# andrewhou1/BlindShadowRemoval

Hardware: AMD Instinct MI355X
Metric: images/sec at 256x256 batch inference (GSC generator forward) (higher is better)
Workload: dtype f32; 1 GPU; BASELINE configs[1]: batch=32 synthetic 256x256x3 per GPU, full GSC generator fp32 (seeded random-init weights in the ckpt-94 variable layout); global_batch=32, height=256, width=256, parallelism=dp1, forwards_in_flight=1, collective=none

## Files before the change

### blindshadowremoval_amd/_lib.py

```python
from __future__ import annotations

import ctypes
import os
from typing import Optional

from . import build as _build
from .build import LIB_PATH

ABI_VERSION = 8
NUM_CLASSES = 7
CLASS_NAMES = ("conv3x3", "convT3x3", "conv1x1", "attention", "conv7", "glue", "convT3x3_ni2")

_lib: Optional[ctypes.CDLL] = None

c_i, c_v, c_sz, c_s = ctypes.c_int, ctypes.c_void_p, ctypes.c_size_t, ctypes.c_char_p
_BS = [c_i, c_i]
_BLOBS = [c_v, c_sz, c_v, c_sz]

SIGNATURES = {
    "bsr_abi_version": (c_i, None),
    "bsr_last_error": (c_s, None),
    "bsr_source_sha": (c_s, None),
    "bsr_create": (c_i, [ctypes.POINTER(c_v), c_i, c_v, c_sz, c_i]),
    "bsr_destroy": (None, [c_v]),
# ... 3 lines not shown
    "bsr_forward_rgb": (c_i, [c_v, c_v, c_v, c_i, c_i, c_i, c_v, c_v]),
    "bsr_workspace_bytes": (c_sz, [c_i, c_i, c_i]),
    "bsr_handle_workspace_bytes": (c_sz, [c_v, c_i, c_i, c_i]),
    "bsr_reserve": (c_i, [c_v, c_i, c_i, c_i]),
    "bsr_probe": (c_i, [c_v, c_s, c_v, c_sz, ctypes.POINTER(c_i * 4), c_v]),
    "bsr_set_timing": (c_i, [c_v, c_i]),
    "bsr_get_timing": (c_i, [c_v, ctypes.POINTER(ctypes.c_float * NUM_CLASSES), ctypes.POINTER(c_i * NUM_CLASSES)]),
    "bsr_timing_launches": (c_i, [c_v]),
    "bsr_timing_entry": (c_i, [c_v, c_i, c_s, c_sz, ctypes.POINTER(ctypes.c_float), ctypes.POINTER(c_i)]),
    "bsr_clock_trace": (c_i, [c_i, c_v, c_i, c_i, c_v, c_v, c_v]),
    "bsr_check_range": (c_i, [c_v, c_v]),
    "bsr_peek_range": (c_i, [c_v]),
    "bsr_debug_attention": (c_i, [c_v, c_v, c_i, c_i, c_v]),
    "bsr_debug_attention_rgb": (c_i, [c_v, c_v, c_i, c_i, c_v]),
    "bsr_debug_attention_dtype": (c_i, [c_v, c_v, c_i, c_i, c_i, c_v]),
    "bsr_debug_attention_qw": (c_i, [c_v, c_v, c_i, c_i, c_i, c_v]),
    "bsr_debug_attention_split": (c_i, [c_v, c_v, c_i, c_i, c_i, c_v]),
    "bsr_debug_attention_kv1": (c_i, [c_v, c_v, c_i, c_i, c_i, c_v]),
    "bsr_debug_split_qkv": (c_i, [c_v, c_v, c_i, c_i, c_v]),
    "bsr_debug_wino_conv": (c_i, [c_v, c_v, c_v, c_v, c_i, c_i, c_i, c_i, c_v]),
    "bsr_debug_wino_filter": (c_i, [c_v, c_v]),
    "bsr_debug_wino_convt": (c_i, [c_v, c_v, c_v, c_v, c_i, c_i, c_i, c_i, c_i, c_i, c_i, c_i, c_v]),
    "bsr_debug_wino_convt_filter": (c_i, [c_v, c_v, c_i]),
    "bsr_debug_keys_compose": (c_i, [c_v, c_v, c_v, c_v]),
    "bsr_debug_values_compose": (c_i, [c_v, c_v, c_v, c_v, c_v, c_v]),
    "bsr_prep_rows": (c_i, [c_i, c_v, c_sz, c_sz, c_sz, c_i, c_i, c_v, c_v, c_v]),
    "bsr_prep_groups": (c_i, [c_i, c_v, c_sz, c_sz, c_sz, c_i, c_i, c_i, c_v, c_v, c_v]),
    "bsr_png_unfilter": (c_i, [c_i, c_v, c_sz, c_sz, c_i, c_v]),
    "bsr_png_unfilter_tall": (c_i, [c_i, c_v, c_sz, c_sz, c_i, c_v]),
    "bsr_png_file_bytes": (c_sz, [c_i, c_i]),
    "bsr_png_scratch_bytes": (c_sz, [c_i]),
    "bsr_png_encode": (c_i, [c_i, c_v, c_i, c_i, c_i, c_v, c_sz, c_v, c_v]),
    "bsr_png_encode_figs": (c_i, [c_i, c_i, c_v, c_v, c_v, c_v, c_v, c_v, c_i, c_i, c_i, c_v, c_sz, c_v, c_v]),
    "bsr_crop_faces": (c_i, [c_i, c_v, c_sz, c_sz, c_i, c_i, c_v]),
    "bsr_paste_faces": (c_i, [c_i, c_v, c_sz, c_sz, c_i, c_i, c_v, c_i, c_v, c_i, c_v, c_i, c_i, c_v]),
    "bsr_ucb_post_scratch_bytes": (c_sz, _BS),
    "bsr_ucb_post": (c_i, [c_i, c_v, c_v, c_v, c_i, c_i, c_v, c_v, c_v, c_v, c_v, c_v]),
    "bsr_ucb_post_rgb_scratch_bytes": (c_sz, _BS),
    "bsr_ucb_post_rgb": (c_i, [c_i, c_v, c_v, c_v, c_i, c_i, c_v, c_v, c_v, c_v, c_v, c_v]),
    "bsr_ucb_post_tsm_scratch_bytes": (c_sz, _BS),
    "bsr_ucb_post_tsm": (c_i, [c_i, c_v, c_v, c_v, c_i, c_i, c_v, c_v, c_v, c_v, c_v, c_v, c_v]),
    "bsr_sfw_score_scratch_bytes": (c_sz, _BS),
    "bsr_sfw_score": (c_i, [c_i, c_v, c_i, c_i, c_v, c_v, c_v, c_v, c_v, c_v, c_v]),
    "bsr_shadow_synth_scratch_bytes": (c_sz, _BS),
    "bsr_shadow_synth": (c_i, [c_i, c_v, c_v, c_v, c_v, c_v, c_sz, c_i, c_i, c_v, c_v, c_v, c_v, c_v, c_v, c_v]),
    "bsr_train_losses_scratch_bytes": (c_sz, _BS),
# ... 160 lines not shown
```

### blindshadowremoval_amd/csrc/bsr_api.hip

```cpp
#include "../../include/bsr_hip.h"

#include <hip/hip_runtime.h>
#include <stdint.h>
#include <stdio.h>
#include <stdlib.h>
#include <string.h>

#include <initializer_list>
#include <string>
#include <type_traits>
#include <unordered_map>
#include <vector>

#include "attention.h"
#include "attention256.h"
#include "attention_h16.h"
#include "conv3_f16.h"
#include "conv_n16.h"
#include "gemm_nloop.h"
#include "glue_kernels.h"
#include "igemm_conv.h"
#include "igemm_h16.h"
#include "png_kernels.h"
#include "prep_kernels.h"
#include "prep_group_kernels.h"
#include "rgb_head.h"
#include "stem7.h"
#include "ucb_kernels.h"
#include "ucb_rgb_kernels.h"
#include "ucb_tsm_kernels.h"
#include "sfw_kernels.h"
#include "wino_conv2.h"
#include "wino_convt.h"
#include "wild_crop_kernels.h"
#include "wild_paste_kernels.h"
#include "shadow_synth_kernels.h"
#include "train_losses_kernels.h"
#include "disc_kernels.h"
#include "disc_grad_kernels.h"
#include "disc_wgrad_kernels.h"
#include "clr_tail_grad_kernels.h"
#include "clr_up_grad_kernels.h"
#include "grey_up_grad_kernels.h"
#include "nonlocal_grad_kernels.h"
#include "bottleneck_grad_kernels.h"
#include "colour_trunk_grad_kernels.h"
#include "lower_trunk_grad_kernels.h"
#include "heads_grad_kernels.h"
#include "vgg_kernels.h"
#include "vgg_grad_kernels.h"

namespace {

thread_local std::string g_last_error;

int fail(int code, const std::string& msg) {
// ... 133 lines not shown
  for (int i = 0; i < v.nblk; ++i) p.r[i] = take(cells * (i < 3 ? v.cs_r : v.cs_h), !v.rgb);
  p.xh = take(cells * v.cs_h, true);
  p.ybuf = take(px * v.cs_y);
  p.qh = take(px * v.cs_qh);
  p.f1 = take(px2 / 16 * 128);
  p.f2 = take(px2 / 4 * 96);
  p.cf = take(px2 * CS_CF);
  p.probe = take(px2 / 64 * 2);
  p.reg32 = take(v.tsm ? cells * 4 : 0);
  p.share = take(v.tsm ? cells * 2 * v.c_r : 0);
  p.yh = take(px1 * 3);
  p.con = take(px1 * 3);
  p.total = off;
  return p;
}

}

struct bsr_handle {
  int device = 0;
  float* d_blob = nullptr;
  float* d_wino = nullptr;
  float* d_winot = nullptr;
  float* d_keys = nullptr;
  float* d_values = nullptr;
  float* att_scratch = nullptr;
  size_t att_scratch_floats = 0;
  std::unordered_map<std::string, LayerW> layers;
  Variant var = kGSC;
  int dtype = BSR_DTYPE_F32;
  float head_bias[2] = {0.f, 0.f};
  const float* tail_w = nullptr;
  const float* clr_gs_w = nullptr;
  float* ws = nullptr;
  size_t ws_floats = 0;
  Plan plan{};
  const float* rgb_tail_w = nullptr;
  const float* rgb_head_b = nullptr;
  int B = 0, H = 0, W = 0;
  bool ran = false;
  bool att_in_lds = false;
  unsigned* range_flag = nullptr;
  bool fuse_heads = true;
  bool conv1_gemm = true;
  bool att_pv1 = false;
  bool conv3_f16 = true;
  bool fuse_attw = true;
  bool wino_conv2 = true;
  bool wino_pairs = true;
  bool wino_convt = true;
  bool keys_conv2 = true;
  bool values_conv2 = true;
  bool att_is_o = false;
  bool timing = false;
  std::vector<hipEvent_t> ev;
  std::vector<int> ev_class;
  std::vector<std::string> ev_name;
  size_t ev_used = 0;
};

namespace {

const char* const kRangeMsg =
    "an activation exceeded the fp16 range (|x| >= 65520) in a forward of this 16-bit-mode handle: its outputs are not trustworthy "
    "(inf / NaN where the fp32 path stays finite).  Re-run those inputs on a BSR_DTYPE_F32 handle; bsr_check_range() clears the condition";

constexpr size_t kWinoFloats = 8 * 16 * 128 * 16;
void wino_filter_transform(const float* direct, float* out) {
  static const double G[4][3] = {{1.0, 0.0, 0.0}, {0.5, 0.5, 0.5}, {0.5, -0.5, 0.5}, {0.0, 0.0, 1.0}};
  for (int k = 0; k < 128; ++k)
    for (int n = 0; n < 128; ++n) {
      double t[4][3];
      for (int x = 0; x < 4; ++x)
// ... 13 lines not shown

constexpr int kWinoTLayers = 3;
const char* const kWinoTNames[kWinoTLayers] = {"up2", "up3", "clr_up3"};
constexpr int kWinoTCin[kWinoTLayers] = {160, 128, 96};
constexpr size_t wino_convt_floats(int cin) { return (size_t)(cin / 16) * 25 * 64 * 16; }
constexpr size_t wino_convt_offset(int layer) { return layer == 0 ? 0 : wino_convt_offset(layer - 1) + wino_convt_floats(kWinoTCin[layer - 1]); }
void wino_convt_filter_transform(const float* direct, float* out, int cin) {
  static const double G[5][3] = {{0.0, 1.0, 0.0}, {0.0, 1.0, 0.0}, {0.0, 0.0, 1.0}, {1.0, 0.0, 1.0}, {1.0, 0.0, 0.0}};
  for (int k = 0; k < cin; ++k)
    for (int n = 0; n < 64; ++n) {
      double t[5][3];
      for (int x = 0; x < 5; ++x)
        for (int b = 0; b < 3; ++b) {
          double acc = 0.0;
          for (int a = 0; a < 3; ++a) acc += G[x][a] * (double)direct[((size_t)((k / 32) * 9 + a * 3 + b) * 64 + n) * 36 + k % 32];
          t[x][b] = acc;
        }
      const int kk = k % 16, g = kk / 8, hh = (kk % 8) / 4, j = kk % 4;
      for (int x = 0; x < 5; ++x)
        for (int y = 0; y < 5; ++y) {
          double acc = 0.0;
          for (int b = 0; b < 3; ++b) acc += t[x][b] * G[y][b];
          out[(((((size_t)(k / 16) * 25 + 5 * x + y) * 2 + n / 32) * 2 + g) * 64 + 32 * hh + n % 32) * 4 + j] = (float)acc;
        }
    }
}

constexpr int kKeysN = 288 + 256, kKeysNPad = kKeysN + 64, kC3qNPad = 768;
constexpr size_t kKeysFloats = (size_t)4 * kKeysNPad * 36 + kKeysNPad;
void keys_compose(const float* c3q_w, const float* c3q_b, float* out_w, float* out_b) {
  auto src = [&](int k, int n) -> const float& { return c3q_w[((size_t)(k / 32) * kC3qNPad + n) * 36 + k % 32]; };
  memset(out_w, 0, (size_t)4 * kKeysNPad * 36 * sizeof(float));
  memset(out_b, 0, kKeysNPad * sizeof(float));
  for (int ch = 0; ch < 4; ++ch) {
    memcpy(out_w + (size_t)ch * kKeysNPad * 36, c3q_w + (size_t)ch * kC3qNPad * 36, (size_t)288 * 36 * sizeof(float));
    memcpy(out_w + ((size_t)ch * kKeysNPad + 416) * 36, c3q_w + ((size_t)ch * kC3qNPad + 544) * 36, (size_t)128 * 36 * sizeof(float));
  }
  memcpy(out_b, c3q_b, 288 * sizeof(float));
  memcpy(out_b + 416, c3q_b + 544, 128 * sizeof(float));
  for (int m = 0; m < 128; ++m) {
    for (int k = 0; k < 128; ++k) {
      double acc = 0.0;
      for (int c = 0; c < 128; ++c) acc += (double)src(k, 288 + c) * (double)src(m, 416 + c);
      out_w[((size_t)(k / 32) * kKeysNPad + 288 + m) * 36 + k % 32] = (float)acc;
    }
    double acc = 0.0;
// ... 301 lines not shown
    end();
    if (fuse) return;
    begin(K_GLUE, "heads_post");
    hipLaunchKernelGGL(bsr::heads_post_kernel, dim3((unsigned)((npix + 255) / 256)), dim3(256), 0, s, qh, inputs, h->head_bias[0], h->head_bias[1], gs,
                       mask22, W, npix);
    check(hipGetLastError(), "heads_post");
    end();
  }

  template <int KH, int KW, bool GS, bool TAIL, int RW>
  void conv16(int cls, const char* name, const float* in, int in_cs, int H, int W, float* out, int out_cs, int act, const float* gs,
              const float* inputs, float* con_rgb, float* dif, float* packed = nullptr) {
    if (rc != BSR_OK) return;
    LayerW l;
    rc = find_layer(h, name, 2, KH * KW, 36, 16, &l);
    if (rc != BSR_OK) return;
    if (l.n_pad != 16) { rc = fail(BSR_ERR_BLOB, std::string("layer '") + name + "' must be packed with n_pad 16"); return; }
    bsr::ConvN16Args a{};
    a.in = in; a.in_cs = in_cs; a.H = H; a.W = W; a.w = l.w; a.bias = l.b; a.out = out; a.out_cs = out_cs; a.act = act;
    a.pad_t = (KH - 1) / 2; a.pad_l = (KW - 1) / 2;
    a.gs = gs; a.w_gs = h->clr_gs_w; a.tail_w = h->tail_w; a.inputs = inputs; a.con_rgb = con_rgb; a.dif = dif; a.packed = packed;
    a.range_flag = h->range_flag;
    if (H % (4 * RW) != 0 || W % 32 != 0) { rc = fail(BSR_ERR_ARG, std::string("layer '") + name + "': image is not a multiple of its tile"); return; }
    begin(cls, name);
    with_dtype(h->dtype, [&](auto prec, auto half) { check(bsr::launch_conv_n16<KH, KW, GS, TAIL, RW, prec.value, half.value>(a, h->B, s), name); });
    end();
  }
};

int grow_workspace(bsr_handle* h, size_t floats, bool device_wide, hipStream_t s) {
  if (floats <= h->ws_floats) return BSR_OK;
  if (device_wide) HIP_TRY(hipDeviceSynchronize());
  else HIP_TRY(hipStreamSynchronize(s));
  if (h->ws) HIP_TRY(hipFree(h->ws));
  h->ws = nullptr;
  h->ws_floats = 0;
  HIP_TRY(hipMalloc(reinterpret_cast<void**>(&h->ws), floats * sizeof(float)));
  h->ws_floats = floats;
  h->B = 0;
  h->ran = false;
  if (device_wide) HIP_TRY(hipMemset(h->ws, 0, floats * sizeof(float)));
  else HIP_TRY(hipMemsetAsync(h->ws, 0, floats * sizeof(float), s));
  return BSR_OK;
}

int ensure_workspace(bsr_handle* h, int B, int H, int W, hipStream_t s) {
// ... 37 lines not shown
  return make_plan(B, H, W, kGSC).total * sizeof(float);
}

int bsr_create(bsr_handle** out, int device, const void* packed_weights, size_t nbytes, int dtype) {
  if (out == nullptr || packed_weights == nullptr) return fail(BSR_ERR_ARG, "bsr_create: null argument");
  *out = nullptr;
  if (dtype != BSR_DTYPE_F32 && dtype != BSR_DTYPE_F16 && dtype != BSR_DTYPE_F32X3)
    return fail(BSR_ERR_ARG, "bsr_create: dtype must be BSR_DTYPE_F32, BSR_DTYPE_F16 or BSR_DTYPE_F32X3");
  if (nbytes < sizeof(BlobHeader)) return fail(BSR_ERR_BLOB, "bsr_create: blob shorter than its header");
  const uint8_t* blob = static_cast<const uint8_t*>(packed_weights);
  BlobHeader hd;
  memcpy(&hd, blob, sizeof hd);
  if (hd.magic != kBlobMagic || hd.version != kBlobVersion) return fail(BSR_ERR_BLOB, "bsr_create: bad blob magic/version");
  if ((int)hd.reserved != dtype) return fail(BSR_ERR_BLOB, "bsr_create: the blob was packed for another dtype (pack_generator(weights, dtype) must match bsr_create's dtype)");
  const size_t table_end = sizeof(BlobHeader) + (size_t)hd.n_entries * sizeof(BlobEntry);
  if (table_end > nbytes) return fail(BSR_ERR_BLOB, "bsr_create: blob entry table exceeds blob size");
  DeviceGuard guard(device);
  HIP_TRY(guard.err);
  bsr_handle* h = new bsr_handle();
  h->device = device;
  h->dtype = dtype;
  h->att_pv1 = dtype == BSR_DTYPE_F16;
  const struct { const char* env; bool* on; } switches[] = {{"BSR_FUSE_HEADS", &h->fuse_heads}, {"BSR_FUSE_ATTW", &h->fuse_attw}, {"BSR_CONV3_F16", &h->conv3_f16},
                                                            {"BSR_CONV1_GEMM", &h->conv1_gemm}, {"BSR_WINO_CONV2", &h->wino_conv2}, {"BSR_WINO_PAIRS", &h->wino_pairs}, {"BSR_WINO_CONVT", &h->wino_convt},
                                                            {"BSR_KEYS_CONV2", &h->keys_conv2}, {"BSR_VALUES_CONV2", &h->values_conv2}};
  for (const auto& sw : switches)
    if (const char* e_ = getenv(sw.env)) *sw.on = atoi(e_) != 0;
  hipError_t e = hipMalloc(reinterpret_cast<void**>(&h->d_blob), nbytes);
  if (e == hipSuccess) e = hipMemcpy(h->d_blob, blob, nbytes, hipMemcpyHostToDevice);
  if (e != hipSuccess) {
    if (h->d_blob) hipFree(h->d_blob);
    delete h;
    return fail(BSR_ERR_HIP, std::string("bsr_create: weight upload: ") + hipGetErrorString(e));
  }
  for (uint32_t i = 0; i < hd.n_entries; ++i) {
    BlobEntry en;
    memcpy(&en, blob + sizeof(BlobHeader) + (size_t)i * sizeof(BlobEntry), sizeof en);
    en.name[sizeof(en.name) - 1] = 0;
    if (en.offset % 16 != 0 || en.offset + en.nfloats * 4 > nbytes) {
      bsr_destroy(h);
      return fail(BSR_ERR_BLOB, std::string("bsr_create: entry '") + en.name + "' is out of bounds or misaligned");
    }
    std::string nm(en.name);
    const float* dptr = reinterpret_cast<const float*>(reinterpret_cast<const uint8_t*>(h->d_blob) + en.offset);
    if (nm == "heads.bias") {
      if (en.nfloats != 2) { bsr_destroy(h); return fail(BSR_ERR_BLOB, "bsr_create: heads.bias must hold 2 floats"); }
      memcpy(h->head_bias, blob + en.offset, 8);
// ... 47 lines not shown
  if (dtype == BSR_DTYPE_F32) {
    std::vector<float> u(6 * kWinoFloats);
    for (int i = 0; i < 6; ++i) {
      char nm[32];
      snprintf(nm, sizeof nm, "res%d.conv2", i);
      LayerW l;
      if (find_layer(h, nm, 4, 9, 36, 128, &l) != BSR_OK || l.n_pad != 128) { bsr_destroy(h); return fail(BSR_ERR_BLOB, std::string("bsr_create: layer '") + nm + "' is not a [4][9][128][36] image"); }
      wino_filter_transform(reinterpret_cast<const float*>(blob + (reinterpret_cast<const uint8_t*>(l.w) - reinterpret_cast<const uint8_t*>(h->d_blob))), u.data() + i * kWinoFloats);
    }
    e = hipMalloc(reinterpret_cast<void**>(&h->d_wino), u.size() * sizeof(float));
    if (e == hipSuccess) e = hipMemcpy(h->d_wino, u.data(), u.size() * sizeof(float), hipMemcpyHostToDevice);
    if (e != hipSuccess) { bsr_destroy(h); return fail(BSR_ERR_HIP, std::string("bsr_create: Winograd weights: ") + hipGetErrorString(e)); }
    if (!h->var.tsm) {
      std::vector<float> ut(wino_convt_offset(kWinoTLayers));
      for (int i = 0; i < kWinoTLayers; ++i) {
        LayerW l;
        if (find_layer(h, kWinoTNames[i], kWinoTCin[i] / 32, 9, 36, 64, &l) != BSR_OK || l.n_pad != 64) { bsr_destroy(h); return fail(BSR_ERR_BLOB, std::string("bsr_create: layer '") + kWinoTNames[i] + "' is not a [Cin / 32][9][64][36] image"); }
        wino_convt_filter_transform(reinterpret_cast<const float*>(blob + (reinterpret_cast<const uint8_t*>(l.w) - reinterpret_cast<const uint8_t*>(h->d_blob))), ut.data() + wino_convt_offset(i), kWinoTCin[i]);
      }
      e = hipMalloc(reinterpret_cast<void**>(&h->d_winot), ut.size() * sizeof(float));
      if (e == hipSuccess) e = hipMemcpy(h->d_winot, ut.data(), ut.size() * sizeof(float), hipMemcpyHostToDevice);
      if (e != hipSuccess) { bsr_destroy(h); return fail(BSR_ERR_HIP, std::string("bsr_create: transposed-layer Winograd weights: ") + hipGetErrorString(e)); }
    }
    std::vector<float> q(6 * kKeysFloats);
    auto host = [&](const float* dev) { return reinterpret_cast<const float*>(blob + (reinterpret_cast<const uint8_t*>(dev) - reinterpret_cast<const uint8_t*>(h->d_blob))); };
    for (int i = 0; i < 6; ++i) {
      char nm[32];
      snprintf(nm, sizeof nm, "res%d.c3q", i);
      LayerW l;
      if (find_layer(h, nm, 4, 1, 36, kC3qNPad, &l) != BSR_OK || l.n_pad != kC3qNPad) { bsr_destroy(h); return fail(BSR_ERR_BLOB, std::string("bsr_create: layer '") + nm + "' is not a [4][1][768][36] image"); }
      keys_compose(host(l.w), host(l.b), q.data() + i * kKeysFloats, q.data() + i * kKeysFloats + (size_t)4 * kKeysNPad * 36);
    }
    e = hipMalloc(reinterpret_cast<void**>(&h->d_keys), q.size() * sizeof(float));
    if (e == hipSuccess) e = hipMemcpy(h->d_keys, q.data(), q.size() * sizeof(float), hipMemcpyHostToDevice);
    if (e != hipSuccess) { bsr_destroy(h); return fail(BSR_ERR_HIP, std::string("bsr_create: composed c3q weights: ") + hipGetErrorString(e)); }
    std::vector<float> v(6 * kValuesFloats);
    for (int i = 0; i < 6; ++i) {
      char nm[32];
      LayerW l, lw;
      snprintf(nm, sizeof nm, "res%d.c3q", i);
      if (find_layer(h, nm, 4, 1, 36, kC3qNPad, &l) != BSR_OK) { bsr_destroy(h); return BSR_ERR_BLOB; }
      snprintf(nm, sizeof nm, "res%d.w", i);
      if (find_layer(h, nm, 4, 1, 36, kWNPad, &lw) != BSR_OK || lw.n_pad != kWNPad) { bsr_destroy(h); return fail(BSR_ERR_BLOB, std::string("bsr_create: layer '") + nm + "' is not a [4][1][384][36] image"); }
      float* vw = v.data() + i * kValuesFloats;
      float* vc = vw + kValuesWFloats;
      float* vg = vc + kValuesC3qFloats;
      const float* kq = q.data() + i * kKeysFloats;
      values_compose(host(l.w), host(l.b), host(lw.w), host(lw.b), vw, vw + (size_t)4 * kWNPad * 36);
      values_cut(kq, kq + (size_t)4 * kKeysNPad * 36, host(l.w), host(l.b), vc, vc + (size_t)4 * kValuesNPad * 36, vg, vg + (size_t)4 * kGProbeNPad * 36);
    }
    e = hipMalloc(reinterpret_cast<void**>(&h->d_values), v.size() * sizeof(float));
    if (e == hipSuccess) e = hipMemcpy(h->d_values, v.data(), v.size() * sizeof(float), hipMemcpyHostToDevice);
    if (e != hipSuccess) { bsr_destroy(h); return fail(BSR_ERR_HIP, std::string("bsr_create: composed w weights: ") + hipGetErrorString(e)); }
  }
  *out = h;
  return BSR_OK;
}

void bsr_destroy(bsr_handle* h) {
  if (h == nullptr) return;
  DeviceGuard guard(h->device);
  for (hipEvent_t e : h->ev) hipEventDestroy(e);
  if (h->ws) hipFree(h->ws);
  if (h->d_blob) hipFree(h->d_blob);
  if (h->d_wino) hipFree(h->d_wino);
  if (h->d_winot) hipFree(h->d_winot);
  if (h->d_keys) hipFree(h->d_keys);
  if (h->d_values) hipFree(h->d_values);
  if (h->att_scratch) hipFree(h->att_scratch);
  if (h->range_flag) hipHostFree(h->range_flag);
  delete h;
}

int bsr_reserve(bsr_handle* h, int B, int H, int W) {
  if (h == nullptr || B <= 0 || H <= 0 || W <= 0) return fail(BSR_ERR_ARG, "bsr_reserve: bad argument");
  DeviceGuard guard(h->device);
  HIP_TRY(guard.err);
  return grow_workspace(h, make_plan(B, H, W, h->var).total, true, nullptr);
}

int bsr_check_range(bsr_handle* h, void* stream) {
  if (h == nullptr) return fail(BSR_ERR_ARG, "bsr_check_range: null handle");
  if (h->range_flag == nullptr) return BSR_OK;
  DeviceGuard guard(h->device);
  HIP_TRY(guard.err);
  HIP_TRY(hipStreamSynchronize(static_cast<hipStream_t>(stream)));
  if (__atomic_exchange_n(h->range_flag, 0u, __ATOMIC_SEQ_CST) == 0u) return BSR_OK;
  return fail(BSR_ERR_RANGE, kRangeMsg);
}
// ... 1299 lines not shown
  std::vector<float> u(wino_convt_floats(cin));
  wino_convt_filter_transform(w_direct, u.data(), cin);
  float* d_u = nullptr;
  HIP_TRY(hipMalloc(reinterpret_cast<void**>(&d_u), u.size() * sizeof(float)));
  hipError_t e = hipMemcpy(d_u, u.data(), u.size() * sizeof(float), hipMemcpyHostToDevice);
  if (e == hipSuccess) {
    bsr::WinoTArgs a{};
    a.in = x; a.out = y; a.w = d_u; a.bias = bias; a.H = H; a.W = W; a.in_cs = in_cs; a.out_cs = out_cs; a.nchunk = cin / 16; a.act = act ? 1 : 0;
    e = bsr::launch_wino_convt(a, B, s);
  }
  if (e == hipSuccess) e = hipStreamSynchronize(s);
  hipFree(d_u);
  HIP_TRY(e);
  return BSR_OK;
}

int bsr_debug_wino_convt_filter(const float* direct, float* out, int cin) {
  if (direct == nullptr || out == nullptr) return fail(BSR_ERR_ARG, "bsr_debug_wino_convt_filter: null argument");
  if (cin <= 0 || cin % 16 != 0) return fail(BSR_ERR_ARG, "bsr_debug_wino_convt_filter: Cin must be a positive multiple of 16");
  wino_convt_filter_transform(direct, out, cin);
  return BSR_OK;
}

int bsr_debug_wino_filter(const float* direct, float* out) {
  if (direct == nullptr || out == nullptr) return fail(BSR_ERR_ARG, "bsr_debug_wino_filter: null argument");
  wino_filter_transform(direct, out);
  return BSR_OK;
}

int bsr_debug_keys_compose(const float* c3q_w, const float* c3q_b, float* out_w, float* out_b) {
  if (c3q_w == nullptr || c3q_b == nullptr || out_w == nullptr || out_b == nullptr) return fail(BSR_ERR_ARG, "bsr_debug_keys_compose: null argument");
  keys_compose(c3q_w, c3q_b, out_w, out_b);
  return BSR_OK;
}

int bsr_debug_values_compose(const float* c3q_w, const float* c3q_b, const float* w_w, const float* w_b, float* out_w, float* out_b) {
  if (c3q_w == nullptr || c3q_b == nullptr || w_w == nullptr || w_b == nullptr || out_w == nullptr || out_b == nullptr)
    return fail(BSR_ERR_ARG, "bsr_debug_values_compose: null argument");
  values_compose(c3q_w, c3q_b, w_w, w_b, out_w, out_b);
  return BSR_OK;
}

int bsr_debug_attention(const float* qkv, float* y, int B, int tokens, void* stream) {
  return bsr_debug_attention_dtype(qkv, y, B, tokens, BSR_DTYPE_F32, stream);
}

// ... 214 lines not shown
```

### blindshadowremoval_amd/pack.py

```python
from __future__ import annotations

import struct
from typing import Dict, List, Tuple

import numpy as np

from .weights import BN_EPS, N_RES, check_weights, detect_variant

BLOB_MAGIC = 0x57525342
BLOB_VERSION = 1
_ENTRY = struct.Struct("<40sQQ4i")
_HEADER = struct.Struct("<4I")

TRANSPOSED = ("up1", "up2", "up3", "clr_up1", "clr_up2", "clr_up3")

DTYPES = {"f32": 0, "f16": 1, "f32x3": 2}
H16_LAYERS = ("down1", "down2", "down3", "up1", "up2", "up3", "clr_up1", "clr_up2", "clr_up3") + tuple("res%d.conv2" % i for i in range(6))
W3_LAYERS = ("up1", "up2", "up3", "clr_up1", "clr_up2", "clr_up3") + tuple("res%d.conv2" % i for i in range(6))
X3_LAYERS = tuple("res%d.%s" % (i, n) for i in range(6) for n in ("conv1", "c3q", "w")) + ("heads", "clr_conv1", "conv1")


def geometry(variant: str = "gsc", dtype: str = "f32") -> Dict[str, Tuple[int, int, int]]:
    if variant == "rgb":
        return geometry_rgb(dtype)
# ... 152 lines not shown
    arr = np.ascontiguousarray(u.reshape(16, k // WINO_CC, WINO_CC, n).transpose(1, 0, 3, 2))
    return arr, bias.astype(np.float32)


WINO_CONVT_BT = np.array([[0.0, 1, 0], [0, 0, 1], [1, -1, 0], [0, 1, 0], [0, 1, -1]])
WINO_CONVT_G = np.array([[0.0, 1, 0], [0, 1, 0], [0, 0, 1], [1, 0, 1], [1, 0, 0]])
WINO_CONVT_AT = np.array([[0.0, 0, 1, 1, 0], [1, 0, 0, 0, 0], [0, 0, 0, 1, -1], [0, 1, 0, 0, 0]])


def wino_convt_filter_transform(kernel_tkn: np.ndarray, dtype=np.float32) -> np.ndarray:
    taps, k, n = kernel_tkn.shape
    assert taps == 9
    g = kernel_tkn.astype(np.float64).reshape(3, 3, k, n)
    return np.einsum("xa,abkn,yb->xykn", WINO_CONVT_G, g, WINO_CONVT_G).reshape(25, k, n).astype(dtype)


def pack_wino_convt(kernel_tkn: np.ndarray, bias: np.ndarray):
    taps, k, n = kernel_tkn.shape
    assert k % WINO_CC == 0 and n == 64
    u = wino_convt_filter_transform(kernel_tkn.astype(np.float32))
    u = u.reshape(25, k // WINO_CC, 2, 2, 4, 2, 32)
    arr = np.ascontiguousarray(u.transpose(1, 0, 5, 2, 3, 6, 4)).reshape(k // WINO_CC, 25, 2, 2, 64, 4)
    return arr, bias.astype(np.float32)


KEYS_N = 288 + 256
KEYS_N_PAD = KEYS_N + 64


def compose_keys(wq: np.ndarray, bq: np.ndarray, wk: np.ndarray):
    wq, wk, bq = wq.astype(np.float64), wk.astype(np.float64), bq.astype(np.float64)
    return wq @ wk.T, bq @ wk.T


def compose_keys_c3q(c3q_w: np.ndarray, c3q_b: np.ndarray):
    assert c3q_w.shape == (4, 1, 768, 36) and c3q_b.shape == (768,)
    kn = c3q_w[:, 0, :, :32].transpose(0, 2, 1).reshape(128, 768)
    a, ab = compose_keys(kn[:, 288:416], c3q_b[288:416], kn[:, 416:544])
    out = np.zeros((4, 1, KEYS_N_PAD, 36), np.float32)
    out[:, :, :288] = c3q_w[:, :, :288]
    out[:, 0, 288:416, :32] = a.astype(np.float32).reshape(4, 32, 128).transpose(0, 2, 1)
    out[:, :, 416:544] = c3q_w[:, :, 544:672]
    b = np.zeros(KEYS_N_PAD, np.float32)
    b[:288], b[288:416], b[416:544] = c3q_b[:288], ab.astype(np.float32), c3q_b[544:672]
    return out, b

# ... 814 lines not shown
```

### include/bsr_hip.h

```cpp
#ifndef BSR_HIP_H_
#define BSR_HIP_H_

#include <stddef.h>

#ifdef __cplusplus
extern "C" {
#endif

typedef struct bsr_handle bsr_handle;

#define BSR_OK 0
#define BSR_ERR_ARG 1
#define BSR_ERR_BLOB 2
#define BSR_ERR_HIP 3
#define BSR_ERR_STATE 4
#define BSR_ERR_RANGE 5

#define BSR_DTYPE_F32 0
#define BSR_DTYPE_F16 1
#define BSR_DTYPE_F32X3 2

int bsr_create(bsr_handle** out, int device, const void* packed_weights, size_t nbytes, int dtype);

int bsr_forward(bsr_handle* h, const float* inputs, const float* uv, int B, int H, int W,
// ... 216 lines not shown
size_t bsr_ucb_post_rgb_scratch_bytes(int B, int S);
int bsr_ucb_post_rgb(int device, const float* rows9, const unsigned char* masks, const float* boxes, int B, int S, float* losses,
                     unsigned char* strips, float* figs, int* status, void* scratch, void* stream);

size_t bsr_sfw_score_scratch_bytes(int B, int S);
int bsr_sfw_score(int device, const float* rows3, int B, int S, float* losses, double* auc, float* pred, float* label, int* status,
                  void* scratch, void* stream);

size_t bsr_ucb_post_tsm_scratch_bytes(int B, int S);
int bsr_ucb_post_tsm(int device, const float* rows, const unsigned char* masks, const float* boxes, int B, int S, float* losses,
                     double* nose_stats, unsigned char* strips, float* figs, int* status, void* scratch, void* stream);

int bsr_debug_attention(const float* qkv, float* y, int B, int tokens, void* stream);
int bsr_debug_attention_rgb(const float* qkv, float* y, int B, int tokens, void* stream);
int bsr_debug_attention_dtype(const float* qkv, float* y, int B, int tokens, int dtype, void* stream);
int bsr_debug_split_qkv(const float* qkv, void* qkv_split, int B, int tokens, void* stream);
int bsr_debug_attention_split(const void* qkv_split, float* y, int B, int tokens, int pv1, void* stream);
int bsr_debug_attention_qw(const float* qkv, float* y, int B, int tokens, int qw, void* stream);
int bsr_debug_wino_conv(const float* x, const float* w, const float* bias, float* y, int B, int H, int W, int nw, void* stream);
int bsr_debug_wino_filter(const float* direct, float* out);
int bsr_debug_wino_convt(const float* x, const float* w_direct, const float* bias, float* y, int B, int H, int W, int cin, int cout, int in_cs,
                         int out_cs, int act, void* stream);
int bsr_debug_wino_convt_filter(const float* direct, float* out, int cin);
int bsr_debug_keys_compose(const float* c3q_w, const float* c3q_b, float* out_w, float* out_b);
int bsr_debug_values_compose(const float* c3q_w, const float* c3q_b, const float* w_w, const float* w_b, float* out_w, float* out_b);
int bsr_debug_attention_kv1(const float* qkv2, float* y, int B, int tokens, int qw, void* stream);

int bsr_clock_trace(int device, unsigned long long* out, int samples, int spin, const int* stop, int* taken, void* stream);

void bsr_destroy(bsr_handle* h);

const char* bsr_last_error(void);

int bsr_abi_version(void);

const char* bsr_source_sha(void);

#ifdef __cplusplus
}
#endif
#endif
```

Baseline: 7368 images/sec.

## Add Winograd F(2x2,3x3) kernel for fp32 colour-tail conv with fused head

Result: faster. 7562 images/sec, median of 6 (+2.6%).

```diff
diff --git a/blindshadowremoval_amd/_lib.py b/blindshadowremoval_amd/_lib.py
--- a/blindshadowremoval_amd/_lib.py
+++ b/blindshadowremoval_amd/_lib.py
@@ -49,6 +49,8 @@
     "bsr_debug_wino_filter": (c_i, [c_v, c_v]),
     "bsr_debug_wino_convt": (c_i, [c_v, c_v, c_v, c_v, c_i, c_i, c_i, c_i, c_i, c_i, c_i, c_i, c_v]),
     "bsr_debug_wino_convt_filter": (c_i, [c_v, c_v, c_i]),
+    "bsr_debug_wino_clr": (c_i, [c_v, c_v, c_i, c_v, c_v, c_v, c_v, c_v, c_v, c_v, c_v, c_i, c_i, c_i, c_i, c_v]),
+    "bsr_debug_wino_clr_filter": (c_i, [c_v, c_v, c_v]),
     "bsr_debug_keys_compose": (c_i, [c_v, c_v, c_v, c_v]),
     "bsr_debug_values_compose": (c_i, [c_v, c_v, c_v, c_v, c_v, c_v]),
     "bsr_prep_rows": (c_i, [c_i, c_v, c_sz, c_sz, c_sz, c_i, c_i, c_v, c_v, c_v]),
diff --git a/blindshadowremoval_amd/csrc/bsr_api.hip b/blindshadowremoval_amd/csrc/bsr_api.hip
--- a/blindshadowremoval_amd/csrc/bsr_api.hip
+++ b/blindshadowremoval_amd/csrc/bsr_api.hip
@@ -32,6 +32,7 @@
 #include "sfw_kernels.h"
 #include "wino_conv2.h"
 #include "wino_convt.h"
+#include "wino_clr.h"
 #include "wild_crop_kernels.h"
 #include "wild_paste_kernels.h"
 #include "shadow_synth_kernels.h"
@@ -211,6 +212,7 @@
   float* d_blob = nullptr;
   float* d_wino = nullptr;
   float* d_winot = nullptr;
+  float* d_wclr = nullptr;
   float* d_keys = nullptr;
   float* d_values = nullptr;
   float* att_scratch = nullptr;
@@ -238,6 +240,7 @@
   bool wino_conv2 = true;
   bool wino_pairs = true;
   bool wino_convt = true;
+  bool wino_clr = true;
   bool keys_conv2 = true;
   bool values_conv2 = true;
   bool att_is_o = false;
@@ -297,6 +300,30 @@
           double acc = 0.0;
           for (int b = 0; b < 3; ++b) acc += t[x][b] * G[y][b];
           out[(((((size_t)(k / 16) * 25 + 5 * x + y) * 2 + n / 32) * 2 + g) * 64 + 32 * hh + n % 32) * 4 + j] = (float)acc;
+        }
+    }
+}
+
+constexpr size_t kWinoClrFloats = bsr::WinoClrCfg::W_FLOATS;
+void wino_clr_filter_transform(const float* direct, const float* w_gs, float* out) {
+  static const double G[4][3] = {{1.0, 0.0, 0.0}, {0.5, 0.5, 0.5}, {0.5, -0.5, 0.5}, {0.0, 0.0, 1.0}};
+  for (int k = 0; k < 65; ++k)
+    for (int n = 0; n < 16; ++n) {
+      double t[4][3];
+      for (int x = 0; x < 4; ++x)
+        for (int b = 0; b < 3; ++b) {
+          double acc = 0.0;
+          for (int a = 0; a < 3; ++a)
+            acc += G[x][a] * (double)(k < 64 ? direct[((size_t)((k / 32) * 9 + a * 3 + b) * 16 + n) * 36 + k % 32] : w_gs[n * 16 + a * 3 + b]);
+          t[x][b] = acc;
+        }
+      for (int x = 0; x < 4; ++x)
+        for (int y = 0; y < 4; ++y) {
+          double acc = 0.0;
+          for (int b = 0; b < 3; ++b) acc += t[x][b] * G[y][b];
+          const int pos = 4 * x + y;
+          if (k < 64) out[((size_t)(pos * 4 + k / 16) * 64 + 16 * ((k % 16) / 4) + n) * 4 + k % 4] = (float)acc;
+          else out[bsr::WinoClrCfg::U_FLOATS + pos * 16 + n] = (float)acc;
         }
     }
 }
@@ -644,6 +671,16 @@
     a.gs = gs; a.w_gs = h->clr_gs_w; a.tail_w = h->tail_w; a.inputs = inputs; a.con_rgb = con_rgb; a.dif = dif; a.packed = packed;
     a.range_flag = h->range_flag;
     if (H % (4 * RW) != 0 || W % 32 != 0) { rc = fail(BSR_ERR_ARG, std::string("layer '") + name + "': image is not a multiple of its tile"); return; }
+    if constexpr (KH == 3 && KW == 3 && GS && TAIL && RW == 2) {
+      if (h->dtype == BSR_DTYPE_F32 && h->wino_clr && h->d_wclr != nullptr) {
+        if (const char* why = bsr::wino_clr_refusal(h->B, H, W, in_cs)) { rc = fail(BSR_ERR_ARG, std::string("layer '") + name + "': " + why); return; }
+        a.w = h->d_wclr;
+        begin(cls, name);
+        check(bsr::launch_wino_clr(a, h->B, s), name);
+        end();
+        return;
+      }
+    }
     begin(cls, name);
     with_dtype(h->dtype, [&](auto prec, auto half) { check(bsr::launch_conv_n16<KH, KW, GS, TAIL, RW, prec.value, half.value>(a, h->B, s), name); });
     end();
@@ -727,7 +764,7 @@
   h->dtype = dtype;
   h->att_pv1 = dtype == BSR_DTYPE_F16;
   const struct { const char* env; bool* on; } switches[] = {{"BSR_FUSE_HEADS", &h->fuse_heads}, {"BSR_FUSE_ATTW", &h->fuse_attw}, {"BSR_CONV3_F16", &h->conv3_f16},
-                                                            {"BSR_CONV1_GEMM", &h->conv1_gemm}, {"BSR_WINO_CONV2", &h->wino_conv2}, {"BSR_WINO_PAIRS", &h->wino_pairs}, {"BSR_WINO_CONVT", &h->wino_convt},
+                                                            {"BSR_CONV1_GEMM", &h->conv1_gemm}, {"BSR_WINO_CONV2", &h->wino_conv2}, {"BSR_WINO_PAIRS", &h->wino_pairs}, {"BSR_WINO_CONVT", &h->wino_convt}, {"BSR_WINO_CLR", &h->wino_clr},
                                                             {"BSR_KEYS_CONV2", &h->keys_conv2}, {"BSR_VALUES_CONV2", &h->values_conv2}};
   for (const auto& sw : switches)
     if (const char* e_ = getenv(sw.env)) *sw.on = atoi(e_) != 0;
@@ -821,6 +858,16 @@
       if (e == hipSuccess) e = hipMemcpy(h->d_winot, ut.data(), ut.size() * sizeof(float), hipMemcpyHostToDevice);
       if (e != hipSuccess) { bsr_destroy(h); return fail(BSR_ERR_HIP, std::string("bsr_create: transposed-layer Winograd weights: ") + hipGetErrorString(e)); }
     }
+    {
+      LayerW l;
+      if (find_layer(h, "clr_conv1", 2, 9, 36, 16, &l) != BSR_OK || l.n_pad != 16) { bsr_destroy(h); return fail(BSR_ERR_BLOB, "bsr_create: layer 'clr_conv1' is not a [2][9][16][36] image"); }
+      std::vector<float> uc(kWinoClrFloats);
+      auto host_of = [&](const float* dev) { return reinterpret_cast<const float*>(blob + (reinterpret_cast<const uint8_t*>(dev) - reinterpret_cast<const uint8_t*>(h->d_blob))); };
+      wino_clr_filter_transform(host_of(l.w), host_of(h->clr_gs_w), uc.data());
+      e = hipMalloc(reinterpret_cast<void**>(&h->d_wclr), uc.size() * sizeof(float));
+      if (e == hipSuccess) e = hipMemcpy(h->d_wclr, uc.data(), uc.size() * sizeof(float), hipMemcpyHostToDevice);
+      if (e != hipSuccess) { bsr_destroy(h); return fail(BSR_ERR_HIP, std::string("bsr_create: colour-tail Winograd weights: ") + hipGetErrorString(e)); }
+    }
     std::vector<float> q(6 * kKeysFloats);
     auto host = [&](const float* dev) { return reinterpret_cast<const float*>(blob + (reinterpret_cast<const uint8_t*>(dev) - reinterpret_cast<const uint8_t*>(h->d_blob))); };
     for (int i = 0; i < 6; ++i) {
@@ -864,6 +911,7 @@
   if (h->d_blob) hipFree(h->d_blob);
   if (h->d_wino) hipFree(h->d_wino);
   if (h->d_winot) hipFree(h->d_winot);
+  if (h->d_wclr) hipFree(h->d_wclr);
   if (h->d_keys) hipFree(h->d_keys);
   if (h->d_values) hipFree(h->d_values);
   if (h->att_scratch) hipFree(h->att_scratch);
@@ -2209,6 +2257,41 @@
   return BSR_OK;
 }
 
+int bsr_debug_wino_clr_filter(const float* direct, const float* w_gs, float* out) {
+  if (direct == nullptr || w_gs == nullptr || out == nullptr) return fail(BSR_ERR_ARG, "bsr_debug_wino_clr_filter: null argument");
+  wino_clr_filter_transform(direct, w_gs, out);
+  return BSR_OK;
+}
+
+int bsr_debug_wino_clr(const float* gs, const float* f, int in_cs, const float* inputs, const float* w_direct, const float* w_gs, const float* bias,
+                       const float* tail_w, float* con_rgb, float* dif, float* packed, int B, int H, int W, int wino, void* stream) {
+  if (gs == nullptr || f == nullptr || inputs == nullptr || w_direct == nullptr || w_gs == nullptr || bias == nullptr || tail_w == nullptr)
+    return fail(BSR_ERR_ARG, "bsr_debug_wino_clr: null argument");
+  if (packed == nullptr && (con_rgb == nullptr || dif == nullptr)) return fail(BSR_ERR_ARG, "bsr_debug_wino_clr: neither packed nor con_rgb | dif given");
+  if (const char* why = bsr::wino_clr_refusal(B, H, W, in_cs)) return fail(BSR_ERR_ARG, std::string("bsr_debug_wino_clr: ") + why);
+  hipStream_t s = static_cast<hipStream_t>(stream);
+  constexpr size_t kDirect = 2 * 9 * 16 * 36, kGs = kDirect, kBias = kGs + 256, kTail = kBias + 16, kU = kTail + 340;
+  std::vector<float> img(kU + kWinoClrFloats, 0.f);
+  memcpy(img.data(), w_direct, kDirect * sizeof(float));
+  memcpy(img.data() + kGs, w_gs, 256 * sizeof(float));
+  memcpy(img.data() + kBias, bias, 16 * sizeof(float));
+  memcpy(img.data() + kTail, tail_w, 337 * sizeof(float));
+  wino_clr_filter_transform(w_direct, w_gs, img.data() + kU);
+  float* d = nullptr;
+  HIP_TRY(hipMalloc(reinterpret_cast<void**>(&d), img.size() * sizeof(float)));
+  hipError_t e = hipMemcpy(d, img.data(), img.size() * sizeof(float), hipMemcpyHostToDevice);
+  if (e == hipSuccess) {
+    bsr::ConvN16Args a{};
+    a.in = f; a.in_cs = in_cs; a.H = H; a.W = W; a.w = wino ? d + kU : d; a.bias = d + kBias; a.act = 1; a.pad_t = 1; a.pad_l = 1;
+    a.gs = gs; a.w_gs = d + kGs; a.tail_w = d + kTail; a.inputs = inputs; a.con_rgb = con_rgb; a.dif = dif; a.packed = packed;
+    e = wino ? bsr::launch_wino_clr(a, B, s) : bsr::launch_conv_n16<3, 3, true, true, 2>(a, B, s);
+  }
+  if (e == hipSuccess) e = hipStreamSynchronize(s);
+  hipFree(d);
+  HIP_TRY(e);
+  return BSR_OK;
+}
+
 int bsr_debug_wino_filter(const float* direct, float* out) {
   if (direct == nullptr || out == nullptr) return fail(BSR_ERR_ARG, "bsr_debug_wino_filter: null argument");
   wino_filter_transform(direct, out);
diff --git a/blindshadowremoval_amd/csrc/wino_clr.h b/blindshadowremoval_amd/csrc/wino_clr.h
--- /dev/null
+++ b/blindshadowremoval_amd/csrc/wino_clr.h
@@ -0,0 +1,275 @@
+#pragma once
+#include <hip/hip_runtime.h>
+
+#include "conv_n16.h"
+
+namespace bsr {
+
+struct WinoClrCfg {
+  static constexpr int TH = 8, TW = 32;
+  static constexpr int U_FLOATS = 16 * 4 * 64 * 4;
+  static constexpr int UGS_FLOATS = 16 * 16;
+  static constexpr int W_FLOATS = U_FLOATS + UGS_FLOATS;
+  static constexpr int TAIL_FLOATS = 340 + 16;
+  static constexpr int SMEM_BYTES = (W_FLOATS + TAIL_FLOATS) * 4;
+  static_assert(2 * SMEM_BYTES <= 160 * 1024, "two workgroups per compute unit");
+};
+
+template <int CTRL>
+__device__ __forceinline__ float wino_clr_from_lane(float old, float src) {
+  return __int_as_float(__builtin_amdgcn_update_dpp(__float_as_int(old), __float_as_int(src), CTRL, 0xf, 0xf, false));
+}
+template <int CTRL>
+__device__ __forceinline__ f32x4 wino_clr_from_lane(const f32x4& old, const f32x4& src) {
+  return f32x4{wino_clr_from_lane<CTRL>(old[0], src[0]), wino_clr_from_lane<CTRL>(old[1], src[1]), wino_clr_from_lane<CTRL>(old[2], src[2]),
+               wino_clr_from_lane<CTRL>(old[3], src[3])};
+}
+
+__global__ __launch_bounds__(256, 2) void wino_clr_kernel(ConvN16Args p) {
+  using C = WinoClrCfg;
+  typedef unsigned u32x2_t __attribute__((ext_vector_type(2)));
+  extern __shared__ __attribute__((aligned(16))) float smem[];
+  float* s_u = smem;
+  float* s_ugs = smem + C::U_FLOATS;
+  float* s_tail = smem + C::W_FLOATS;
+
+  const int tid = threadIdx.x, lane = tid & 63;
+  const int wave = __builtin_amdgcn_readfirstlane(tid >> 6);
+  const int r = lane & 15, q = lane >> 4;
+
+  struct Tile { int img, y0, x0; };
+  const int ntiles = p.tiles_x * p.tiles_y * p.batch;
+  auto decode = [&](int t) {
+    Tile d;
+    d.x0 = (t % p.tiles_x) * C::TW;
+    t /= p.tiles_x;
+    d.y0 = (t % p.tiles_y) * C::TH;
+    d.img = t / p.tiles_y;
+    return d;
+  };
+
+  const __amdgpu_buffer_rsrc_t no_rsrc = __builtin_amdgcn_make_buffer_rsrc(const_cast<float*>(p.in), 0, 0, 0x00020000);
+  auto pick = [&](bool ok, const __amdgpu_buffer_rsrc_t& a) { return ok ? a : no_rsrc; };
+  auto edge_col = [&](const Tile& d) { return r == 0 && d.x0 > 0 ? 0 : r == 15 && d.x0 + C::TW < p.W ? C::TW + 1 : -1; };
+  auto fetch_f = [&](const Tile& d, int g, f32x4 (&regs)[12]) {
+    const int iy0 = d.y0 + 2 * wave - 1, ix0 = d.x0 - 1;
+    const __amdgpu_buffer_rsrc_t rs = make_rsrc(p.in + (((ptrdiff_t)d.img * p.H + iy0) * p.W + ix0) * p.in_cs);
+    const __amdgpu_buffer_rsrc_t rs0 = pick(iy0 >= 0, rs), rs3 = pick(iy0 + 3 < p.H, rs);
+    const int ec = edge_col(d);
+    const unsigned voff[3] = {(unsigned)((2 * r + 1) * p.in_cs + 4 * q) * 4u, (unsigned)((2 * r + 2) * p.in_cs + 4 * q) * 4u,
+                              ec >= 0 ? (unsigned)(ec * p.in_cs + 4 * q) * 4u : kLaneOff};
+#pragma unroll
+    for (int a = 0; a < 4; ++a)
+#pragma unroll
+      for (int b = 0; b < 3; ++b)
+        regs[3 * a + b] = __builtin_bit_cast(f32x4, __builtin_amdgcn_raw_buffer_load_b128(a == 0 ? rs0 : a == 3 ? rs3 : rs, voff[b],
+                                                                                           (unsigned)(a * p.W * p.in_cs + g * 16) * 4u, 0));
+  };
+  const __amdgpu_buffer_rsrc_t no_gs = __builtin_amdgcn_make_buffer_rsrc(const_cast<float*>(p.gs), 0, 0, 0x00020000);
+  auto fetch_gs = [&](const Tile& d, float (&regs)[12]) {
+    const int iy0 = d.y0 + 2 * wave - 1, ix0 = d.x0 - 1;
+    const __amdgpu_buffer_rsrc_t rs = make_rsrc(p.gs + ((ptrdiff_t)d.img * p.H + iy0) * p.W + ix0);
+    const __amdgpu_buffer_rsrc_t rs0 = iy0 >= 0 ? rs : no_gs, rs3 = iy0 + 3 < p.H ? rs : no_gs;
+    const int ec = edge_col(d);
+    const unsigned voff[3] = {q == 0 ? (unsigned)(2 * r + 1) * 4u : kLaneOff, q == 0 ? (unsigned)(2 * r + 2) * 4u : kLaneOff,
+                              q == 0 && ec >= 0 ? (unsigned)ec * 4u : kLaneOff};
+#pragma unroll
+    for (int a = 0; a < 4; ++a)
+#pragma unroll
+      for (int b = 0; b < 3; ++b)
+        regs[3 * a + b] = __uint_as_float(__builtin_amdgcn_raw_buffer_load_b32(a == 0 ? rs0 : a == 3 ? rs3 : rs, voff[b], (unsigned)(a * p.W) * 4u, 0));
+  };
+  auto transform = [&](const auto (&d)[12], auto (&v)[16]) {
+#pragma unroll
+    for (int b = 0; b < 3; ++b) {
+      v[b] = d[b] - d[6 + b];
+      v[4 + b] = d[3 + b] + d[6 + b];
+      v[8 + b] = d[6 + b] - d[3 + b];
+      v[12 + b] = d[3 + b] - d[9 + b];
+    }
+#pragma unroll
+    for (int x = 0; x < 4; ++x) {
+      const auto c1 = v[4 * x], c2 = v[4 * x + 1], ce = v[4 * x + 2];
+      const auto c0 = wino_clr_from_lane<0x111>(ce, c2), c3 = wino_clr_from_lane<0x101>(ce, c1);
+      v[4 * x] = c0 - c2; v[4 * x + 1] = c1 + c2; v[4 * x + 2] = c2 - c1; v[4 * x + 3] = c1 - c3;
+    }
+  };
+
+  int tile = (int)blockIdx.x;
+  Tile cur = decode(tile < ntiles ? tile : 0);
+  f32x4 ld[12];
+  fetch_f(cur, 0, ld);
+  for (int i = tid; i < C::W_FLOATS / 4; i += 256) reinterpret_cast<f32x4*>(smem)[i] = reinterpret_cast<const f32x4*>(p.w)[i];
+  for (int i = tid; i < 337; i += 256) s_tail[i] = p.tail_w[i];
+  if (tid < 16) s_tail[340 + tid] = p.bias[tid];
+  __syncthreads();
+
+  const float* u_lane = s_u + lane * 4;
+  auto read_u = [&](int pos, int g) { return *reinterpret_cast<const f32x4*>(u_lane + (pos * 4 + g) * 256); };
+
+  for (; tile < ntiles; tile += (int)gridDim.x) {
+    const int tile_n = tile + (int)gridDim.x;
+    const bool has_next = tile_n < ntiles;
+    const Tile nxt = decode(has_next ? tile_n : tile);
+    f32x4 acc[16];
+#pragma unroll
+    for (int i = 0; i < 16; ++i) acc[i] = f32x4{0.f, 0.f, 0.f, 0.f};
+    float gl[12];
+
+#pragma unroll
+    for (int g = 0; g < 4; ++g) {
+      f32x4 v[16];
+      transform(ld, v);
+      if (g < 3) {
+        fetch_f(cur, g + 1, ld);
+      } else {
+        fetch_gs(cur, gl);
+        if (has_next) fetch_f(nxt, 0, ld);
+      }
+      __builtin_amdgcn_sched_barrier(0);
+      f32x4 af[2][2];
+      af[0][0] = read_u(0, g);
+      af[0][1] = read_u(1, g);
+#pragma unroll
+      for (int pp = 0; pp < 8; ++pp) {
+        const int cu = pp & 1, nx = cu ^ 1;
+        if (pp + 1 < 8) {
+          af[nx][0] = read_u(2 * pp + 2, g);
+          af[nx][1] = read_u(2 * pp + 3, g);
+        }
+        __builtin_amdgcn_sched_barrier(0);
+#pragma unroll
+        for (int j = 0; j < 4; ++j)
+#pragma unroll
+          for (int hh = 0; hh < 2; ++hh)
+            acc[2 * pp + hh] = __builtin_amdgcn_mfma_f32_16x16x4f32(af[cu][hh][j], v[2 * pp + hh][j], acc[2 * pp + hh], 0, 0, 0);
+        __builtin_amdgcn_sched_barrier(0);
+      }
+    }
+    {
+      float vg[16];
+      transform(gl, vg);
+      float ag[16];
+#pragma unroll
+      for (int pos = 0; pos < 16; ++pos) ag[pos] = s_ugs[pos * 16 + r];
+      __builtin_amdgcn_sched_barrier(0);
+#pragma unroll
+      for (int pos = 0; pos < 16; ++pos) acc[pos] = __builtin_amdgcn_mfma_f32_16x16x4f32(ag[pos], vg[pos], acc[pos], 0, 0, 0);
+      __builtin_amdgcn_sched_barrier(0);
+    }
+
+    const size_t pix0 = ((size_t)cur.img * p.H + cur.y0 + 2 * wave) * p.W + cur.x0;
+    u32x2_t tin[2][3];
+    {
+      const __amdgpu_buffer_rsrc_t rs = make_rsrc(p.inputs + pix0 * 3);
+      const unsigned voff = q == 0 ? (unsigned)(2 * r * 3) * 4u : kLaneOff;
+#pragma unroll
+      for (int dy = 0; dy < 2; ++dy)
+#pragma unroll
+        for (int e = 0; e < 3; ++e) tin[dy][e] = __builtin_amdgcn_raw_buffer_load_b64(rs, voff, (unsigned)(dy * p.W * 3 + 2 * e) * 4u, 0);
+    }
+    float tw2[4], tw3[4];
+#pragma unroll
+    for (int e = 0; e < 4; ++e) {
+      tw2[e] = s_tail[(4 * q + e) * 16 + r];
+      tw3[e] = s_tail[272 + (4 * q + e) * 3 + (r < 3 ? r : 0)];
+    }
+    const f32x4 tb2 = *reinterpret_cast<const f32x4*>(s_tail + 256 + 4 * q);
+    const f32x4 b4 = *reinterpret_cast<const f32x4*>(s_tail + 340 + 4 * q);
+    float tb3[3];
+#pragma unroll
+    for (int c = 0; c < 3; ++c) tb3[c] = s_tail[320 + c];
+
+    f32x4 y[4];
+    {
+      f32x4 t[2][4];
+#pragma unroll
+      for (int nu = 0; nu < 4; ++nu) {
+        t[0][nu] = (acc[nu] + acc[4 + nu]) + acc[8 + nu];
+        t[1][nu] = (acc[4 + nu] - acc[8 + nu]) - acc[12 + nu];
+      }
+#pragma unroll
+      for (int dy = 0; dy < 2; ++dy) {
+        y[2 * dy] = (t[dy][0] + t[dy][1]) + t[dy][2];
+        y[2 * dy + 1] = (t[dy][1] - t[dy][2]) - t[dy][3];
+      }
+    }
+    f32x4 a3[4];
+#pragma unroll
+    for (int px = 0; px < 4; ++px) {
+      f32x4 v = y[px] + b4;
+      if (p.act) {
+#pragma unroll
+        for (int e = 0; e < 4; e += 2) {
+          const f32x2 z = leaky_relu2(f32x2{v[e], v[e + 1]});
+          v[e] = z[0];
+          v[e + 1] = z[1];
+        }
+      }
+      f32x4 a2 = tb2;
+#pragma unroll
+      for (int e = 0; e < 4; ++e) a2 = __builtin_amdgcn_mfma_f32_16x16x4f32(tw2[e], v[e], a2, 0, 0, 0);
+#pragma unroll
+      for (int e = 0; e < 4; e += 2) {
+        const f32x2 z = leaky_relu2(f32x2{a2[e], a2[e + 1]});
+        a2[e] = z[0];
+        a2[e + 1] = z[1];
+      }
+      a3[px] = f32x4{0.f, 0.f, 0.f, 0.f};
+#pragma unroll
+      for (int e = 0; e < 4; ++e) a3[px] = __builtin_amdgcn_mfma_f32_16x16x4f32(r < 3 ? tw3[e] : 0.f, a2[e], a3[px], 0, 0, 0);
+    }
+    if (q == 0) {
+#pragma clang fp contract(off)
+#pragma unroll
+      for (int px = 0; px < 4; ++px) {
+        const int dy = px >> 1, dx = px & 1;
+        const size_t pix = pix0 + (size_t)dy * p.W + 2 * r + dx;
+        const float in0 = __uint_as_float(dx ? tin[dy][1][1] : tin[dy][0][0]);
+        const float in1 = __uint_as_float(dx ? tin[dy][2][0] : tin[dy][0][1]);
+        const float in2 = __uint_as_float(dx ? tin[dy][2][1] : tin[dy][1][0]);
+        const float cr = a3[px][0] + tb3[0], cg = a3[px][1] + tb3[1], cb = a3[px][2] + tb3[2];
+        const float g1 = (cr * 0.2989f + cg * 0.5870f) + cb * 0.1140f;
+        const float g0 = (in0 * 0.2989f + in1 * 0.5870f) + in2 * 0.1140f;
+        if (p.packed != nullptr) {
+          *reinterpret_cast<f32x4*>(p.packed + pix * 4) = f32x4{cr, cg, cb, g1 - g0};
+        } else {
+          p.con_rgb[pix * 3 + 0] = cr;
+          p.con_rgb[pix * 3 + 1] = cg;
+          p.con_rgb[pix * 3 + 2] = cb;
+          p.dif[pix] = g1 - g0;
+        }
+      }
+    }
+    cur = nxt;
+  }
+}
+
+inline const char* wino_clr_refusal(int batch, int H, int W, int in_cs) {
+  if (batch <= 0 || H <= 0 || W <= 0) return "empty tensor";
+  if (H % WinoClrCfg::TH != 0 || W % WinoClrCfg::TW != 0) return "image is not a multiple of its 8x32 tile";
+  if (in_cs < 64 || in_cs % 4 != 0) return "channel stride must be a multiple of 4, at least 64";
+  if ((long long)4 * (W + 2) * in_cs * 4 >= (1LL << 31)) return "image too wide for 32-bit offsets";
+  if ((long long)batch * (H / WinoClrCfg::TH) * (W / WinoClrCfg::TW) >= (1LL << 31)) return "too many tiles";
+  return nullptr;
+}
+
+inline hipError_t launch_wino_clr(ConvN16Args a, int batch, hipStream_t stream) {
+  using C = WinoClrCfg;
+  static PerDeviceOnce once;
+  const int dev = PerDeviceOnce::current();
+  if (dev < 0 || !once.done[dev]) {
+    hipError_t e = hipFuncSetAttribute(reinterpret_cast<const void*>(wino_clr_kernel), hipFuncAttributeMaxDynamicSharedMemorySize, C::SMEM_BYTES);
+    if (e != hipSuccess) return e;
+    if (dev >= 0) once.done[dev] = true;
+  }
+  a.tiles_x = a.W / C::TW;
+  a.tiles_y = a.H / C::TH;
+  a.batch = batch;
+  const int ntiles = a.tiles_x * a.tiles_y * batch;
+  const int resident = 2 * device_cu_count();
+  hipLaunchKernelGGL(wino_clr_kernel, dim3(ntiles < resident ? ntiles : resident), dim3(256), C::SMEM_BYTES, stream, a);
+  return hipGetLastError();
+}
+
+}
diff --git a/blindshadowremoval_amd/pack.py b/blindshadowremoval_amd/pack.py
--- a/blindshadowremoval_amd/pack.py
+++ b/blindshadowremoval_amd/pack.py
@@ -198,6 +198,15 @@
     u = u.reshape(25, k // WINO_CC, 2, 2, 4, 2, 32)
     arr = np.ascontiguousarray(u.transpose(1, 0, 5, 2, 3, 6, 4)).reshape(k // WINO_CC, 25, 2, 2, 64, 4)
     return arr, bias.astype(np.float32)
+
+
+def pack_wino_clr(kernel_tkn: np.ndarray, gs_tn: np.ndarray) -> np.ndarray:
+    taps, k, n = kernel_tkn.shape
+    assert (taps, k, n) == (9, 64, 16) and gs_tn.shape == (9, 16)
+    u = wino_filter_transform(kernel_tkn.astype(np.float32))
+    u = u.reshape(16, 4, 4, 4, 16).transpose(0, 1, 2, 4, 3)
+    ugs = wino_filter_transform(gs_tn.astype(np.float32).reshape(9, 1, 16))
+    return np.concatenate([np.ascontiguousarray(u).reshape(-1), ugs.reshape(-1)])
 
 
 KEYS_N = 288 + 256
diff --git a/include/bsr_hip.h b/include/bsr_hip.h
--- a/include/bsr_hip.h
+++ b/include/bsr_hip.h
@@ -262,6 +262,9 @@
 int bsr_debug_wino_convt(const float* x, const float* w_direct, const float* bias, float* y, int B, int H, int W, int cin, int cout, int in_cs,
                          int out_cs, int act, void* stream);
 int bsr_debug_wino_convt_filter(const float* direct, float* out, int cin);
+int bsr_debug_wino_clr(const float* gs, const float* f, int in_cs, const float* inputs, const float* w_direct, const float* w_gs, const float* bias,
+                       const float* tail_w, float* con_rgb, float* dif, float* packed, int B, int H, int W, int wino, void* stream);
+int bsr_debug_wino_clr_filter(const float* direct, const float* w_gs, float* out);
 int bsr_debug_keys_compose(const float* c3q_w, const float* c3q_b, float* out_w, float* out_b);
 int bsr_debug_values_compose(const float* c3q_w, const float* c3q_b, const float* w_w, const float* w_b, float* out_w, float* out_b);
 int bsr_debug_attention_kv1(const float* qkv2, float* y, int B, int tokens, int qw, void* stream);
```
